# andrewendlinger/xmris

Measured on AMD Instinct MI355X. Metric: spectra/sec (zero_fill->apodize->FFT->autophase), n_time=4096; HBM-roofline %, higher is better.
Workload: dtype f32

## Files before the change

### xmris_amd/csrc/xm_zf2p.h

```cpp
#pragma once
#include "xm_kernels.h"

enum { ZF2P_LOAD16 = 1, ZF2P_NT = 2, ZF2P_QUEUE = 8, ZF2P_EST = 16, ZF2P_CAND = 32, ZF2P_IN64 = 64 };
constexpr int ZF2P_CAND_CAP = 16;
constexpr int ZF2P_CAND_KMAX = 16384;
constexpr int ZF2P_CAND_ROWS = 1, ZF2P_CAND_EST = 1 + ZF2P_CAND_CAP, ZF2P_CAND_COUNT = 1 + 2 * ZF2P_CAND_CAP,
              ZF2P_CAND_TOP = ZF2P_CAND_COUNT + 1, ZF2P_CAND_BITMAP = ZF2P_CAND_TOP + 1;
constexpr size_t zf2p_cand_lds_bytes() { return (ZF2P_CAND_BITMAP + ZF2P_CAND_KMAX / 32) * sizeof(unsigned); }

constexpr int xm_ilog2(int v) {
  int s = 0;
  while ((1 << s) < v) ++s;
  return s;
}

template <class PL, bool L16>
constexpr int zf2p_pad_shift() {
  if (!L16) return -1;
  return PL::radix(0) == 8 ? 4 : xm_ilog2(2 * PL::radix(0));
}

template <class PL, int MODE, int OPT>
__global__ __launch_bounds__(PL::NT, (zf2_waves<float, PL>())) void k_zf2p(PipeArgs<float> A) {
  using T = float;
  using V = xm_f2;
  constexpr unsigned N = 2 * PL::N, NT = PL::NT;
  constexpr int P = PL::P;
  constexpr bool WRITE = (MODE & ZF2_WRITE) != 0, PHASE = (MODE & ZF2_PHASE) != 0, AMAX = (MODE & ZF2_AMAX) != 0;
  constexpr bool RAMP = (MODE & ZF2_RAMP) != 0;
  constexpr bool L16 = (OPT & ZF2P_LOAD16) != 0;
  constexpr int AUX = (OPT & ZF2P_NT) ? 2 : 0;
  constexpr bool EST = (OPT & ZF2P_EST) != 0, CAND = (OPT & ZF2P_CAND) != 0, IN64 = (OPT & ZF2P_IN64) != 0;
  static_assert(!EST || (NT == XM_WAVE && AMAX && !WRITE), "the per-row estimate is stored by the row's one wave");
  static_assert(!CAND || (AMAX && !WRITE && (OPT & ZF2P_QUEUE) == 0), "candidates: maxima only, static order");
  static_assert(!(IN64 && L16), "pair loads are complex64 loads");
  static_assert(!(PHASE && RAMP), "phase table and ramp are exclusive");
  static_assert(!RAMP || WRITE, "a ramp needs an output");
  static_assert(P % 2 == 0 && NT >= XM_WAVE, "pair loads need an even number of points per thread, whole waves");
  using FFT = BlockFFT<V, PL, zf2p_pad_shift<PL, L16>()>;
  using HT = HotTw<T, PL, RAMP>;
  extern __shared__ __attribute__((aligned(16))) char xm_smem[];
  Cx<V>* lds = reinterpret_cast<Cx<V>*>(xm_smem);
  Cx<T>* mid = reinterpret_cast<Cx<T>*>(lds + FFT::lds_elems());
  T* red_v = reinterpret_cast<T*>(mid + HT::mid_lds_size());
  int* red_i = reinterpret_cast<int*>(red_v + NT / XM_WAVE + 1);
  unsigned* lds_next = reinterpret_cast<unsigned*>(red_i + NT / XM_WAVE + 1);
  constexpr bool QUEUE = (OPT & ZF2P_QUEUE) != 0;
  const unsigned t = threadIdx.x;
  const unsigned lane = t & (XM_WAVE - 1), half = lane >> 5;
  const unsigned col = L16 ? (t & ~(XM_WAVE - 1u)) + 2u * (lane & 31u) + half : t;

  long long n_rows = A.n_batch;
  unsigned* cand = lds_next + ZF2P_CAND_ROWS;
  const unsigned n_in = (unsigned)A.n_in;
  if constexpr (CAND) {
    float* cand_e = reinterpret_cast<float*>(lds_next + ZF2P_CAND_EST);
    unsigned* cand_n = lds_next + ZF2P_CAND_COUNT;
    unsigned* top_bits = lds_next + ZF2P_CAND_TOP;
    unsigned* bitmap = lds_next + ZF2P_CAND_BITMAP;
    const unsigned G = gridDim.x, b = blockIdx.x;
    const unsigned kmax = (unsigned)((A.n_batch + G - 1) / G);
    for (unsigned i = t; i < (kmax + 31u) / 32u; i += NT) bitmap[i] = 0u;
    if (t < XM_WAVE) {
      const unsigned long long k = __hip_atomic_load(A.gkey_in + t * XM_KEY_STRIDE, __ATOMIC_RELAXED, __HIP_MEMORY_SCOPE_AGENT);
      const unsigned hi = wave_reduce_u32<true>((unsigned)(k >> 32));
      if (t == 0) *top_bits = hi;
    }
    __syncthreads();
    const float thr = A.band2 * __uint_as_float(*top_bits);
    for (unsigned k = t; k < kmax; k += NT) {
      const long long r = (long long)k * G + (b + 37u * k) % G;
      if (r < A.n_batch) {
        const float e = A.est[r];
        if (e >= thr || e != e) atomicOr(&bitmap[k >> 5], 1u << (k & 31u));
      }
    }
    __syncthreads();
    if (t == 0) {
      unsigned n = 0;
      for (unsigned w = 0; w < (kmax + 31u) / 32u; ++w) {
        unsigned bits = bitmap[w];
        while (bits) {
          const unsigned k = w * 32u + (unsigned)__builtin_ctz(bits);
          bits &= bits - 1u;
          const unsigned r = (unsigned)((long long)k * G + (b + 37u * k) % G);
          float e = A.est[r];
          e = e != e ? __builtin_inff() : e;
          unsigned pos = n;
          while (pos > 0 && cand_e[pos - 1] < e) --pos;
          if (pos >= (unsigned)ZF2P_CAND_CAP) continue;
          const unsigned top = n < (unsigned)ZF2P_CAND_CAP ? n : (unsigned)ZF2P_CAND_CAP - 1u;
          for (unsigned i = top; i > pos; --i) {
            cand[i] = cand[i - 1];
            cand_e[i] = cand_e[i - 1];
          }
          cand[pos] = r;
          cand_e[pos] = e;
          n = n < (unsigned)ZF2P_CAND_CAP ? n + 1u : n;
        }
      }
      *cand_n = n;
    }
    __syncthreads();
    n_rows = (long long)(unsigned)__builtin_amdgcn_readfirstlane((int)*cand_n);
  }
  const bool live = !CAND || n_rows > 0;

  HT tw;
  tw.mid = HT::mid_in_lds() ? mid : A.tw;
  if (live) {
    tw.load(A.tw, (int)t);
    for (unsigned i = t; i < (unsigned)HT::mid_lds_size(); i += NT) mid[i] = A.tw[i];
  }
  if constexpr (RAMP) {
    double sn, cs;
    sincos(A.ramp_db * (double)(2u * t), &sn, &cs);
    tw.fold(mk<T>((T)cs, (T)sn));
  }
  Cx<T> rot = live ? A.aux[col] : mk<T>(T(0), T(0));
  if constexpr (RAMP) rot = rot * mk<T>(A.ramp_e[0], A.ramp_e[1]);
  const unsigned coff = col - (unsigned)A.pad_left;
  T w[P];
#pragma unroll
  for (int q = 0; q < P; ++q) {
    const bool ok = live && (coff + NT * q) < n_in;
    w[q] = ok ? (A.window ? A.window[col + NT * q] * A.scale : A.scale) : T(0);
  }
  __syncthreads();

  constexpr int NRAW = L16 ? P / 2 : P;
  typedef unsigned raw_t __attribute__((ext_vector_type((L16 || IN64) ? 4 : 2)));
  raw_t raw[NRAW];
  const unsigned e0 = (t & ~(XM_WAVE - 1u)) + 2u * (lane & 31u) + NT * half - (unsigned)A.pad_left;
  auto fetch = [&](long long s2, unsigned ee0, unsigned cc, unsigned nin) {
    constexpr size_t EB = IN64 ? 16u : 8u;
    const char* __restrict__ row = reinterpret_cast<const char*>(A.in) + (size_t)(s2 * A.in_stride) * EB;
    if constexpr (L16) {
#pragma unroll
      for (int j = 0; j < P / 2; ++j) {
        const unsigned e = min(ee0 + 2u * NT * j, nin - 2u);
        raw[j] = __builtin_nontemporal_load(reinterpret_cast<const raw_t*>(row + (size_t)e * 8u));
      }
    } else {
#pragma unroll
      for (int q = 0; q < P; ++q) {
        const unsigned e = min(cc + NT * q, nin - 1u);
        raw[q] = *reinterpret_cast<const raw_t*>(row + (size_t)e * EB);
      }
    }
  };
  unsigned best_key = 0, best_row = 0;
  bool have = false;
  auto rowid = [&](long long v) -> long long {
    if constexpr (CAND) return (long long)(unsigned)__builtin_amdgcn_readfirstlane((int)cand[v]);
    else return v;
  };
  unsigned gb_seen = 0;
  auto next_live = [&](long long v) -> long long {
    if constexpr (CAND) {
      const float* cand_e = reinterpret_cast<const float*>(lds_next + ZF2P_CAND_EST);
      const unsigned gb = wave_reduce_u32<true>(__hip_atomic_load(A.gbest + lane * (2u * XM_KEY_STRIDE), __ATOMIC_RELAXED,
                                                                  __HIP_MEMORY_SCOPE_AGENT));
      gb_seen = gb;
      const float lim = A.band2 * __uint_as_float(gb);
      while (v < n_rows && __uint_as_float((unsigned)__builtin_amdgcn_readfirstlane((int)__float_as_uint(cand_e[v]))) < lim) ++v;
    }
    return v;
  };
  const long long ch = (!CAND && A.queue_chunk > 0) ? A.queue_chunk : 1;
  const long long c_first = CAND ? 0 : blockIdx.x, c_step = CAND ? 1 : gridDim.x;
  long long c_cur = c_first, c_nxt = c_cur + c_step, c_nn = c_nxt + c_step;
  long long s = c_cur * ch;
  unsigned off = 0;
  if constexpr (CAND) {
    if (n_rows > 0) {
      const float* cand_e = reinterpret_cast<const float*>(lds_next + ZF2P_CAND_EST);
      const float top = __uint_as_float((unsigned)__builtin_amdgcn_readfirstlane((int)__float_as_uint(cand_e[0])));
      const float emax2 = __uint_as_float((unsigned)__builtin_amdgcn_readfirstlane((int)lds_next[ZF2P_CAND_TOP]));
      if (top < 0.81f * emax2) {
#pragma unroll 1
        for (int i = 0; i < 3; ++i) __builtin_amdgcn_s_sleep(127);
        if (t < XM_WAVE) {
          const long long nx = next_live(0);
          if (t == 0u) *lds_next = (unsigned)nx;
        }
        __syncthreads();
        s = (long long)(unsigned)__builtin_amdgcn_readfirstlane((int)*lds_next);
        __syncthreads();
      }
    }
  }
  if (s < n_rows) fetch(rowid(s), e0, coff, n_in);
  if constexpr (QUEUE) {
    if (t == 0) *lds_next = atomicAdd(A.queue, 1u) + gridDim.x;
    __syncthreads();
    c_nxt = (long long)(unsigned)__builtin_amdgcn_readfirstlane((int)*lds_next);
    __syncthreads();
  }

  while (s < n_rows) {
    const bool chunk_end = (off + 1 == (unsigned)ch) || (s + 1 >= n_rows);
    long long s_nxt = chunk_end ? c_nxt * ch : s + 1;
    unsigned tt = t, cc = col, sh = (unsigned)A.out_shift, nin = n_in, pl = (unsigned)A.pad_left, ee0 = e0;
    asm volatile("" : "+v"(tt));
    asm volatile("" : "+v"(cc));
    asm volatile("" : "+v"(ee0));
    asm volatile("" : "+s"(sh));
    asm volatile("" : "+s"(nin));
    asm volatile("" : "+s"(pl));

    Cx<T> xr[P];
    if constexpr (L16) {
#pragma unroll
      for (int j = 0; j < P / 2; ++j) {
        const auto re = __builtin_amdgcn_permlane32_swap(raw[j].x, raw[j].z, false, false);
        const auto im = __builtin_amdgcn_permlane32_swap(raw[j].y, raw[j].w, false, false);
        xr[2 * j] = mk<T>(__uint_as_float(re[0]), __uint_as_float(im[0]));
        xr[2 * j + 1] = mk<T>(__uint_as_float(re[1]), __uint_as_float(im[1]));
      }
    } else if constexpr (IN64) {
#pragma unroll
      for (int q = 0; q < P; ++q) {
        Cx<double> d;
        __builtin_memcpy(&d, &raw[q], 16);
        xr[q] = mk<T>((T)d.re, (T)d.im);
      }
    } else {
#pragma unroll
      for (int q = 0; q < P; ++q) xr[q] = mk<T>(__uint_as_float(raw[q].x), __uint_as_float(raw[q].y));
    }
    Cx<V> v[P];
    static_for<0, P>([&](auto qc) {
      constexpr int q = decltype(qc)::value;
      const Cx<T> e = xr[q] * w[q];
      const Cx<T> o = mul_w<q, 2 * P, T>(e * rot);
      v[q].re = V{e.re, o.re};
      v[q].im = V{e.im, o.im};
    });
    if constexpr (!CAND) {
      if (s_nxt < n_rows) fetch(rowid(s_nxt), ee0, cc - pl, nin);
    }
    if constexpr (CAND) {
      FFT::run_cols(v, lds, tw, (int)tt, (int)cc, [&]() {
        if (tt < XM_WAVE) {
          const long long nx = next_live(s + 1);
          if (tt == 0u) *lds_next = (unsigned)nx;
        }
      });
      s_nxt = (long long)(unsigned)__builtin_amdgcn_readfirstlane((int)*lds_next);
      if (s_nxt < n_rows) fetch(rowid(s_nxt), ee0, cc - pl, nin);
    } else if constexpr (QUEUE) {
      const bool claim = off == 0u;
      unsigned ticket = 0;
      if (claim && tt == 0u) ticket = atomicAdd(A.queue, 1u) + gridDim.x;
      FFT::run_cols(v, lds, tw, (int)tt, (int)cc, [&]() {
        if (claim && tt == 0u) *lds_next = ticket;
      });
      if (claim) c_nn = (long long)(unsigned)__builtin_amdgcn_readfirstlane((int)*lds_next);
    } else {
      FFT::run_cols(v, lds, tw, (int)tt, (int)cc);
    }

    const unsigned t2 = 2u * tt;
    if constexpr (AMAX) {
      T bv = T(-1);
#pragma unroll
      for (int q = 0; q < P; ++q) {
        const V m2 = v[q].re * v[q].re + v[q].im * v[q].im;
        bv = fmax(bv, fmax(m2.x, m2.y));
      }
      bv = amax_nan_if_unset(bv);
      if (A.amax_value_only) {
        const unsigned key = wave_reduce_u32<true>(__float_as_uint(bv));
        if (A.gkey) {
          const unsigned r = (unsigned)rowid(s);
          const bool take = !have || key > best_key || (CAND && key == best_key && r < best_row);
          if constexpr (CAND) {
            if (lane == 0u && key > gb_seen) atomicMax(A.gbest + (blockIdx.x % XM_KEY_SLOTS) * (2u * XM_KEY_STRIDE), key);
          }
          best_key = take ? key : best_key;
          best_row = take ? r : best_row;
          have = true;
          if constexpr (EST) {
            if (lane == 0u) A.est[r] = __uint_as_float(key);
          }
        } else {
          if ((tt & (XM_WAVE - 1)) == 0u) atomicMax(reinterpret_cast<unsigned*>(A.absmax2 + s), key);
          if (tt == 0u) A.argidx[s] = 0;
        }
      } else {
        int bi = 0;
        if (!A.amax_value_only) {
          bi = 0x7fffffff;
          const bool all_nan = bv != bv;
#pragma unroll
          for (int q = 0; q < P; ++q) {
            const int k0 = (int)(((2u * NT * q + sh) & (N - 1u)) + t2);
            const V m2 = v[q].re * v[q].re + v[q].im * v[q].im;
            bi = min(bi, ((m2.x == bv) | all_nan) ? k0 : 0x7fffffff);
            bi = min(bi, ((m2.y == bv) | all_nan) ? k0 + 1 : 0x7fffffff);
          }
        }
        amax_reduce_store<T, (int)NT>(bv, bi, (int)tt, true, s, A.absmax2, A.argidx, red_v, red_i);
      }
    }
    if constexpr (WRITE) {
      Cx<T>* __restrict__ orow = A.out + s * (long long)N;
      const __amdgpu_buffer_rsrc_t rph = xm_rsrc(A.phase, PHASE ? N * 8u : 0u);
      typedef const T __attribute__((address_space(4))) * kptr_t;
      kptr_t rc = (kptr_t)((const char __attribute__((address_space(4)))*)__builtin_amdgcn_kernarg_segment_ptr() +
                           __builtin_offsetof(PipeArgs<T>, ramp_c));
      asm volatile("" : "+s"(rc));
      static_for<0, P>([&](auto qc) {
        constexpr int q = decltype(qc)::value;
        const unsigned base = (2u * NT * q + sh) & (N - 1u);
        const __amdgpu_buffer_rsrc_t rout = xm_rsrc(orow + base, 2u * NT * 8u);
        Cx<V> y = v[q];
        if constexpr (RAMP) {
          const V cr = V{rc[2 * q], rc[2 * q]}, ci = V{rc[2 * q + 1], rc[2 * q + 1]};
          y.re = __builtin_elementwise_fma(v[q].re, cr, -(v[q].im * ci));
          y.im = __builtin_elementwise_fma(v[q].re, ci, v[q].im * cr);
        } else if constexpr (PHASE) {
          const CxPair<T> ph = buf_load(rph, t2 * 8u, base * 8u, (CxPair<T>*)nullptr);
          const V cr = V{ph.a.re, ph.b.re}, ci = V{ph.a.im, ph.b.im};
          y.re = __builtin_elementwise_fma(v[q].re, cr, -(v[q].im * ci));
          y.im = __builtin_elementwise_fma(v[q].re, ci, v[q].im * cr);
        }
        xm_u4 u;
        u.x = __float_as_uint(y.re.x);
        u.y = __float_as_uint(y.im.x);
        u.z = __float_as_uint(y.re.y);
        u.w = __float_as_uint(y.im.y);
        __builtin_amdgcn_raw_buffer_store_b128(u, rout, t2 * 8u, 0, AUX);
      });
    }
    if (chunk_end) {
      c_cur = c_nxt;
      c_nxt = c_nn;
      if constexpr (!QUEUE) c_nn = c_nxt + c_step;
      off = 0;
    } else {
      ++off;
    }
    s = s_nxt;
  }
  if constexpr (AMAX) {
    if (A.gkey && have && lane == 0u)
      atomicMax(A.gkey + (blockIdx.x % XM_KEY_SLOTS) * XM_KEY_STRIDE,
                ((unsigned long long)best_key << 32) | (unsigned long long)(0xffffffffu - best_row));
  }
  if constexpr (QUEUE || CAND || (AMAX && WRITE)) {
    bool decode = false;
    if constexpr (AMAX) decode = A.gkey && (A.key_result || (CAND && A.take_flat));
    if (decode) {
      asm volatile("s_waitcnt vmcnt(0)" ::: "memory");
      __syncthreads();
    }
    unsigned last = 0;
    if (t == 0) {
      const unsigned d = atomicAdd(A.queue + 1, 1u);
      last = d == gridDim.x - 1u;
      if (last) {
        __hip_atomic_store(A.queue, 0u, __ATOMIC_RELAXED, __HIP_MEMORY_SCOPE_AGENT);
        __hip_atomic_store(A.queue + 1, 0u, __ATOMIC_RELAXED, __HIP_MEMORY_SCOPE_AGENT);
      }
      if constexpr (CAND) *lds_next = last;
    }
    if constexpr (AMAX) {
      if (decode && t < XM_WAVE) {
        last = (unsigned)__builtin_amdgcn_readfirstlane((int)last);
        if (last) {
          unsigned long long k = __hip_atomic_load(A.gkey + t * XM_KEY_STRIDE, __ATOMIC_RELAXED, __HIP_MEMORY_SCOPE_AGENT);
          __hip_atomic_store(A.gkey + t * XM_KEY_STRIDE, 0ull, __ATOMIC_RELAXED, __HIP_MEMORY_SCOPE_AGENT);
          if constexpr (CAND) {
            __hip_atomic_store(A.gkey_in + t * XM_KEY_STRIDE, 0ull, __ATOMIC_RELAXED, __HIP_MEMORY_SCOPE_AGENT);
            __hip_atomic_store(A.gbest + t * (2u * XM_KEY_STRIDE), 0u, __ATOMIC_RELAXED, __HIP_MEMORY_SCOPE_AGENT);
          }
#pragma unroll
          for (int m = XM_WAVE / 2; m >= 1; m >>= 1) {
            const unsigned hi = (unsigned)__shfl_xor((int)(k >> 32), m, XM_WAVE), lo = (unsigned)__shfl_xor((int)(unsigned)k, m, XM_WAVE);
            const unsigned long long o = ((unsigned long long)hi << 32) | lo;
            k = o > k ? o : k;
          }
          if (t == 0) {
            const unsigned row = k ? 0xffffffffu - (unsigned)(k & 0xffffffffu) : 0u;
            if (A.key_result) {
              A.key_result->max2 = __uint_as_float((unsigned)(k >> 32));
              A.key_result->flat = (long long)row * (long long)N;
            }
            if constexpr (CAND) {
              if (A.take_max2) A.take_max2[0] = __uint_as_float((unsigned)(k >> 32));
              A.take_flat[0] = (long long)row * (long long)N;
              cand[0] = row;
            }
          }
        }
      }
      if constexpr (CAND) {
        if (decode) {
          __syncthreads();
          if (*lds_next != 0u && A.take_row) {
            const size_t r = (size_t)cand[0] * (size_t)A.in_stride;
            for (unsigned j = t; j < n_in; j += NT) {
              if constexpr (IN64) {
                A.take_row[j] = reinterpret_cast<const Cx<double>*>(A.in)[r + j];
              } else {
                const Cx<T> x = A.in[r + j];
                A.take_row[j] = mk<double>((double)x.re, (double)x.im);
              }
            }
          }
        }
      }
    }
  }
}
```

Baseline: 58.03 million.

## Recompute top estimated row first in candidate pass, speculatively gather its input

The candidate refinement pass now first recomputes only the row that held the previous global maximum. It uses that exact value to tighten the threshold before picking candidates, which replaces the old sleep-and-poll wait when the top estimate looked weak. One block speculatively copies that row's input to the output early, so the final decode can skip the gather when the winner is unchanged. This adds an extra block-wide sync and reduction after the first row, plus a second candidate scan, and the bookkeeping for which block records keys becomes more intricate.

```diff
diff --git a/xmris_amd/csrc/xm_zf2p.h b/xmris_amd/csrc/xm_zf2p.h
--- a/xmris_amd/csrc/xm_zf2p.h
+++ b/xmris_amd/csrc/xm_zf2p.h
@@ -5,7 +5,7 @@
 constexpr int ZF2P_CAND_CAP = 16;
 constexpr int ZF2P_CAND_KMAX = 16384;
 constexpr int ZF2P_CAND_ROWS = 1, ZF2P_CAND_EST = 1 + ZF2P_CAND_CAP, ZF2P_CAND_COUNT = 1 + 2 * ZF2P_CAND_CAP,
-              ZF2P_CAND_TOP = ZF2P_CAND_COUNT + 1, ZF2P_CAND_BITMAP = ZF2P_CAND_TOP + 1;
+              ZF2P_CAND_BITMAP = ZF2P_CAND_COUNT + 1;
 constexpr size_t zf2p_cand_lds_bytes() { return (ZF2P_CAND_BITMAP + ZF2P_CAND_KMAX / 32) * sizeof(unsigned); }
 
 constexpr int xm_ilog2(int v) {
@@ -53,24 +53,15 @@
   long long n_rows = A.n_batch;
   unsigned* cand = lds_next + ZF2P_CAND_ROWS;
   const unsigned n_in = (unsigned)A.n_in;
-  if constexpr (CAND) {
+  auto pick_candidates = [&](float thr, unsigned skip) -> long long {
     float* cand_e = reinterpret_cast<float*>(lds_next + ZF2P_CAND_EST);
     unsigned* cand_n = lds_next + ZF2P_CAND_COUNT;
-    unsigned* top_bits = lds_next + ZF2P_CAND_TOP;
     unsigned* bitmap = lds_next + ZF2P_CAND_BITMAP;
     const unsigned G = gridDim.x, b = blockIdx.x;
     const unsigned kmax = (unsigned)((A.n_batch + G - 1) / G);
-    for (unsigned i = t; i < (kmax + 31u) / 32u; i += NT) bitmap[i] = 0u;
-    if (t < XM_WAVE) {
-      const unsigned long long k = __hip_atomic_load(A.gkey_in + t * XM_KEY_STRIDE, __ATOMIC_RELAXED, __HIP_MEMORY_SCOPE_AGENT);
-      const unsigned hi = wave_reduce_u32<true>((unsigned)(k >> 32));
-      if (t == 0) *top_bits = hi;
-    }
-    __syncthreads();
-    const float thr = A.band2 * __uint_as_float(*top_bits);
     for (unsigned k = t; k < kmax; k += NT) {
       const long long r = (long long)k * G + (b + 37u * k) % G;
-      if (r < A.n_batch) {
+      if (r < A.n_batch && (unsigned)r != skip) {
         const float e = A.est[r];
         if (e >= thr || e != e) atomicOr(&bitmap[k >> 5], 1u << (k & 31u));
       }
@@ -102,7 +93,25 @@
       *cand_n = n;
     }
     __syncthreads();
-    n_rows = (long long)(unsigned)__builtin_amdgcn_readfirstlane((int)*cand_n);
+    return (long long)(unsigned)__builtin_amdgcn_readfirstlane((int)*cand_n);
+  };
+  unsigned est_top = 0, row_top = 0xffffffffu, top_seen = 0;
+  bool top_pass = false;
+  if constexpr (CAND) {
+    unsigned* bitmap = lds_next + ZF2P_CAND_BITMAP;
+    const unsigned kmax = (unsigned)((A.n_batch + gridDim.x - 1) / gridDim.x);
+    for (unsigned i = t; i < (kmax + 31u) / 32u; i += NT) bitmap[i] = 0u;
+    const unsigned long long k = wave_reduce_u64_max(
+        __hip_atomic_load(A.gkey_in + lane * XM_KEY_STRIDE, __ATOMIC_RELAXED, __HIP_MEMORY_SCOPE_AGENT));
+    est_top = (unsigned)(k >> 32);
+    top_pass = est_top > 0u && est_top < 0x7f800000u && (long long)(0xffffffffu - (unsigned)k) < A.n_batch;
+    if (top_pass) {
+      row_top = 0xffffffffu - (unsigned)k;
+      if (t == 0) cand[0] = row_top;
+      n_rows = 1;
+    }
+    __syncthreads();
+    if (!top_pass) n_rows = pick_candidates(A.band2 * __uint_as_float(est_top), 0xffffffffu);
   }
   const bool live = !CAND || n_rows > 0;
 
@@ -155,12 +164,24 @@
     if constexpr (CAND) return (long long)(unsigned)__builtin_amdgcn_readfirstlane((int)cand[v]);
     else return v;
   };
+  auto gather_row = [&](unsigned row) {
+    const size_t r = (size_t)row * (size_t)A.in_stride;
+    for (unsigned j = t; j < n_in; j += NT) {
+      if constexpr (IN64) {
+        A.take_row[j] = reinterpret_cast<const Cx<double>*>(A.in)[r + j];
+      } else {
+        const Cx<T> x = A.in[r + j];
+        A.take_row[j] = mk<double>((double)x.re, (double)x.im);
+      }
+    }
+  };
   unsigned gb_seen = 0;
   auto next_live = [&](long long v) -> long long {
     if constexpr (CAND) {
       const float* cand_e = reinterpret_cast<const float*>(lds_next + ZF2P_CAND_EST);
-      const unsigned gb = wave_reduce_u32<true>(__hip_atomic_load(A.gbest + lane * (2u * XM_KEY_STRIDE), __ATOMIC_RELAXED,
-                                                                  __HIP_MEMORY_SCOPE_AGENT));
+      unsigned gb = wave_reduce_u32<true>(__hip_atomic_load(A.gbest + lane * (2u * XM_KEY_STRIDE), __ATOMIC_RELAXED,
+                                                            __HIP_MEMORY_SCOPE_AGENT));
+      gb = gb > top_seen ? gb : top_seen;
       gb_seen = gb;
       const float lim = A.band2 * __uint_as_float(gb);
       while (v < n_rows && __uint_as_float((unsigned)__builtin_amdgcn_readfirstlane((int)__float_as_uint(cand_e[v]))) < lim) ++v;
@@ -172,25 +193,12 @@
   long long c_cur = c_first, c_nxt = c_cur + c_step, c_nn = c_nxt + c_step;
   long long s = c_cur * ch;
   unsigned off = 0;
+  if (s < n_rows) fetch(rowid(s), e0, coff, n_in);
+  bool top_gathered = false;
   if constexpr (CAND) {
-    if (n_rows > 0) {
-      const float* cand_e = reinterpret_cast<const float*>(lds_next + ZF2P_CAND_EST);
-      const float top = __uint_as_float((unsigned)__builtin_amdgcn_readfirstlane((int)__float_as_uint(cand_e[0])));
-      const float emax2 = __uint_as_float((unsigned)__builtin_amdgcn_readfirstlane((int)lds_next[ZF2P_CAND_TOP]));
-      if (top < 0.81f * emax2) {
-#pragma unroll 1
-        for (int i = 0; i < 3; ++i) __builtin_amdgcn_s_sleep(127);
-        if (t < XM_WAVE) {
-          const long long nx = next_live(0);
-          if (t == 0u) *lds_next = (unsigned)nx;
-        }
-        __syncthreads();
-        s = (long long)(unsigned)__builtin_amdgcn_readfirstlane((int)*lds_next);
-        __syncthreads();
-      }
-    }
-  }
-  if (s < n_rows) fetch(rowid(s), e0, coff, n_in);
+    top_gathered = top_pass && A.gkey && (A.key_result || A.take_flat) && A.take_row;
+    if (top_gathered && blockIdx.x == (gridDim.x > 1u ? 1u : 0u)) gather_row(row_top);
+  }
   if constexpr (QUEUE) {
     if (t == 0) *lds_next = atomicAdd(A.queue, 1u) + gridDim.x;
     __syncthreads();
@@ -242,13 +250,15 @@
     }
     if constexpr (CAND) {
       FFT::run_cols(v, lds, tw, (int)tt, (int)cc, [&]() {
-        if (tt < XM_WAVE) {
+        if (!top_pass && tt < XM_WAVE) {
           const long long nx = next_live(s + 1);
           if (tt == 0u) *lds_next = (unsigned)nx;
         }
       });
-      s_nxt = (long long)(unsigned)__builtin_amdgcn_readfirstlane((int)*lds_next);
-      if (s_nxt < n_rows) fetch(rowid(s_nxt), ee0, cc - pl, nin);
+      if (!top_pass) {
+        s_nxt = (long long)(unsigned)__builtin_amdgcn_readfirstlane((int)*lds_next);
+        if (s_nxt < n_rows) fetch(rowid(s_nxt), ee0, cc - pl, nin);
+      }
     } else if constexpr (QUEUE) {
       const bool claim = off == 0u;
       unsigned ticket = 0;
@@ -274,15 +284,39 @@
         const unsigned key = wave_reduce_u32<true>(__float_as_uint(bv));
         if (A.gkey) {
           const unsigned r = (unsigned)rowid(s);
-          const bool take = !have || key > best_key || (CAND && key == best_key && r < best_row);
+          bool book = true;
+          if constexpr (CAND) book = !top_pass || blockIdx.x == 0u;
+          if (book) {
+            const bool take = !have || key > best_key || (CAND && key == best_key && r < best_row);
+            if constexpr (CAND) {
+              if (lane == 0u && key > gb_seen) atomicMax(A.gbest + (blockIdx.x % XM_KEY_SLOTS) * (2u * XM_KEY_STRIDE), key);
+            }
+            best_key = take ? key : best_key;
+            best_row = take ? r : best_row;
+            have = true;
+            if constexpr (EST) {
+              if (lane == 0u) A.est[r] = __uint_as_float(key);
+            }
+          }
           if constexpr (CAND) {
-            if (lane == 0u && key > gb_seen) atomicMax(A.gbest + (blockIdx.x % XM_KEY_SLOTS) * (2u * XM_KEY_STRIDE), key);
-          }
-          best_key = take ? key : best_key;
-          best_row = take ? r : best_row;
-          have = true;
-          if constexpr (EST) {
-            if (lane == 0u) A.est[r] = __uint_as_float(key);
+            if (top_pass) {
+              unsigned* red_u = reinterpret_cast<unsigned*>(red_v);
+              if (lane == 0u) red_u[tt / XM_WAVE] = key;
+              __syncthreads();
+              unsigned m = 0u;
+              for (unsigned i = 0; i < NT / XM_WAVE; ++i) m = red_u[i] > m ? red_u[i] : m;
+              top_seen = (unsigned)__builtin_amdgcn_readfirstlane((int)m);
+              top_pass = false;
+              n_rows = pick_candidates(A.band2 * fmaxf(__uint_as_float(est_top), __uint_as_float(top_seen)), row_top);
+              if (tt < XM_WAVE) {
+                const long long nx = next_live(0);
+                if (tt == 0u) *lds_next = (unsigned)nx;
+              }
+              __syncthreads();
+              s_nxt = (long long)(unsigned)__builtin_amdgcn_readfirstlane((int)*lds_next);
+              __syncthreads();
+              if (s_nxt < n_rows) fetch(rowid(s_nxt), ee0, cc - pl, nin);
+            }
           }
         } else {
           if ((tt & (XM_WAVE - 1)) == 0u) atomicMax(reinterpret_cast<unsigned*>(A.absmax2 + s), key);
@@ -399,17 +433,7 @@
       if constexpr (CAND) {
         if (decode) {
           __syncthreads();
-          if (*lds_next != 0u && A.take_row) {
-            const size_t r = (size_t)cand[0] * (size_t)A.in_stride;
-            for (unsigned j = t; j < n_in; j += NT) {
-              if constexpr (IN64) {
-                A.take_row[j] = reinterpret_cast<const Cx<double>*>(A.in)[r + j];
-              } else {
-                const Cx<T> x = A.in[r + j];
-                A.take_row[j] = mk<double>((double)x.re, (double)x.im);
-              }
-            }
-          }
+          if (*lds_next != 0u && A.take_row && !(top_gathered && cand[0] == row_top)) gather_row(cand[0]);
         }
       }
     }
```

After: 58.72 million, median of 6. 1.2% higher.
